# HaSai666/rec_pangu

Hardware: AMD Instinct MI355X
Metric: samples/sec DeepFM Criteo-shape bsz=65536/GPU (train step: fwd+bwd+dense Adam+zero_grad) (higher is better)
Workload: dtype f32

## Files before the change

### rec_pangu_amd/csrc/embed.hip

```cpp
#include "common.h"
#include <cstdlib>
#include "bfsplit.h"

struct IdxPtrs {
    const int64_t *p[RP_MAX_FIELDS];
};
struct DensePtrs {
    const float *p[RP_MAX_FIELDS];
};

template <int VEC>
struct Vec;
template <>
struct Vec<4> {
    typedef f32x4 T;
    static __device__ __forceinline__ T load(const float *p) { return *reinterpret_cast<const f32x4 *>(p); }
    static __device__ __forceinline__ void store(float *p, T v) { *reinterpret_cast<f32x4 *>(p) = v; }
    static __device__ __forceinline__ T zero() { return f32x4{0.f, 0.f, 0.f, 0.f}; }
    static __device__ __forceinline__ float hsum(T v) { return (v.x + v.y) + (v.z + v.w); }
};
template <>
struct Vec<1> {
    typedef float T;
    static __device__ __forceinline__ T load(const float *p) { return *p; }
    static __device__ __forceinline__ void store(float *p, T v) { *p = v; }
    static __device__ __forceinline__ T zero() { return 0.f; }
    static __device__ __forceinline__ float hsum(T v) { return v; }
};

template <int TPR, int VEC>
__global__ __launch_bounds__(256) void embed_gather_fwd_kernel(
    const float *__restrict__ arena, const int64_t *__restrict__ row_base, const int64_t *__restrict__ row_count,
    IdxPtrs idx, int F, DensePtrs dense, int ND, int64_t B, int D, float *__restrict__ x, int64_t ldx,
    float *__restrict__ fm_out, float *__restrict__ sum_out, int32_t *__restrict__ keys_out,
    int32_t *__restrict__ err_flag) {
    typedef Vec<VEC> V;
    constexpr int SPB = 256 / TPR;
    const int t = threadIdx.x % TPR;
    const int64_t b = (int64_t)blockIdx.x * SPB + threadIdx.x / TPR;
    if (b >= B) return;
    float *xrow = x + b * ldx;
    float fm_acc = 0.f;
    for (int c = t * VEC; c < D; c += TPR * VEC) {
        typename V::T s = V::zero(), q = V::zero();
#pragma unroll 4
        for (int f = 0; f < F; ++f) {
            int64_t id = idx.p[f][b];
            if (id < 0 || id >= row_count[f]) {
                *err_flag = 1;
                id = 0;
            }
            const int64_t key = row_base[f] + id;
            const typename V::T v = V::load(arena + key * D + c);
            V::store(xrow + (int64_t)f * D + c, v);
            s += v;
            q += v * v;
            if (keys_out != nullptr && c == 0) keys_out[(int64_t)f * B + b] = (int32_t)key;
        }
        if (sum_out != nullptr) V::store(sum_out + b * D + c, s);
        fm_acc += V::hsum(s * s - q);
    }
    const int64_t dense0 = (int64_t)F * D;
    for (int j = t; j < ND; j += TPR) xrow[dense0 + j] = dense.p[j][b];
    for (int64_t j = dense0 + ND + t; j < ldx; j += TPR) xrow[j] = 0.f;
    if (fm_out != nullptr) {
#pragma unroll
        for (int o = TPR / 2; o > 0; o >>= 1) fm_acc += __shfl_xor(fm_acc, o, TPR);
        if (t == 0) fm_out[b] = 0.5f * fm_acc;
    }
}

#define RP_SEG 8
template <int TPR, int VEC, bool LEVEL1 = false, bool POOL = false>
__global__ __launch_bounds__(256) void embed_grad_reduce_kernel(
    const int32_t *__restrict__ sk, const int32_t *__restrict__ sp, int64_t n, int Bi, int D,
    const float *__restrict__ dx, int64_t ldx, const float *__restrict__ gfm, const float *__restrict__ sum_in,
    const float *__restrict__ arena, float *__restrict__ G, int accumulate, float *__restrict__ gpiece,
    int32_t *__restrict__ gkey, const int32_t *__restrict__ bag_of = nullptr, const float *__restrict__ scale = nullptr) {
    typedef Vec<VEC> V;
    constexpr int GPB = 256 / TPR;
    constexpr int W = TPR * VEC;
    __shared__ __attribute__((aligned(16))) float piece[GPB][2][W];
    __shared__ int32_t pkey[GPB][2];
    __shared__ int32_t pcont[GPB];
    const int t = threadIdx.x % TPR, grp = threadIdx.x / TPR;
    const int64_t start = ((int64_t)blockIdx.x * GPB + grp) * RP_SEG;
    const bool active = start < n;
    const int cnt = active ? (int)((n - start) < RP_SEG ? (n - start) : RP_SEG) : 0;
    int32_t k[RP_SEG];
    int bb[RP_SEG], ff[RP_SEG];
#pragma unroll
    for (int j = 0; j < RP_SEG; ++j) {
        const bool ok = j < cnt;
        k[j] = ok ? sk[start + j] : -1;
        if (LEVEL1) {
            ff[j] = 0;
            bb[j] = (int)(start + j);
        } else if (POOL) {
            const int32_t p = ok ? sp[start + j] : 0;
            ff[j] = 0;
            bb[j] = bag_of ? (ok ? bag_of[p] : 0) : p / Bi;
        } else {
            const int32_t p = ok ? sp[start + j] : 0;
            ff[j] = p / Bi;
            bb[j] = p - ff[j] * Bi;
        }
    }
    const int32_t kprev = (active && start > 0) ? sk[start - 1] : -1;
    const int32_t knext = (active && start + cnt < n) ? sk[start + cnt] : -1;
    if (LEVEL1) {
        bool any = false;
#pragma unroll
        for (int j = 0; j < RP_SEG; ++j) any |= k[j] >= 0;
        if (!__syncthreads_or((int)any)) {
            if (threadIdx.x == 0) {
                gkey[2 * (int64_t)blockIdx.x] = -1;
                gkey[2 * (int64_t)blockIdx.x + 1] = -1;
            }
            return;
        }
    }
    float *hp = gpiece + (int64_t)blockIdx.x * 2 * D, *tp = hp + D;
    for (int c0 = 0; c0 < D; c0 += W) {
        const int c = c0 + t * VEC;
        const bool col_ok = c < D;
        typename V::T r[RP_SEG], w[RP_SEG];
        float gf[RP_SEG];
#pragma unroll
        for (int j = 0; j < RP_SEG; ++j) {
            r[j] = V::zero();
            w[j] = V::zero();
            gf[j] = 0.f;
            if (j < cnt && col_ok && !(LEVEL1 && k[j] < 0)) {
                if (dx != nullptr) r[j] = V::load(dx + (int64_t)bb[j] * ldx + (int64_t)ff[j] * D + c);
                if (POOL && scale != nullptr) r[j] = r[j] * V::load(scale + (int64_t)bb[j] * D + c);
                if (gfm != nullptr) {
                    gf[j] = gfm[bb[j]];
                    if (sum_in != nullptr) r[j] += gf[j] * V::load(sum_in + (int64_t)bb[j] * D + c);
                    if (j + 1 >= cnt || k[j + 1] != k[j]) w[j] = V::load(arena + (int64_t)k[j] * D + c);
                }
            }
        }
        if (t == 0) {
            pkey[grp][0] = -1;
            pkey[grp][1] = -1;
            pcont[grp] = 0;
        }
        typename V::T acc = V::zero();
        float gs = 0.f;
        bool run_head = (k[0] != kprev);
#pragma unroll
        for (int j = 0; j < RP_SEG; ++j) {
            if (j < cnt) {
                acc += r[j];
                gs += gf[j];
                const bool last_of_run = (j + 1 < cnt) ? (k[j + 1] != k[j]) : true;
                if (last_of_run) {
                    const bool run_ends_here = (j + 1 < cnt) ? true : (k[j] != knext);
                    if (gfm != nullptr) acc -= gs * w[j];
                    if (LEVEL1 && k[j] < 0) {
                    } else if (run_head && run_ends_here) {
                        if (col_ok) {
                            float *dst = G + (int64_t)k[j] * D + c;
                            V::store(dst, accumulate ? V::load(dst) + acc : acc);
                        }
                    } else {
                        const int slot = run_head ? 1 : 0;
                        V::store(&piece[grp][slot][t * VEC], acc);
                        if (t == 0) {
                            pkey[grp][slot] = k[j];
                            if (!run_ends_here) pcont[grp] = 1;
                        }
                    }
                    acc = V::zero();
                    gs = 0.f;
                    run_head = true;
                }
            }
        }
        __syncthreads();
        if (grp == 0) {
            const bool head_open = pkey[0][0] >= 0;
            int last_g = -1;
            for (int g2 = GPB - 1; g2 >= 0; --g2)
                if (pkey[g2][0] >= 0 || pkey[g2][1] >= 0) {
                    last_g = g2;
                    break;
                }
            const int64_t wg_end = ((int64_t)blockIdx.x + 1) * GPB * RP_SEG;
            const int last_active = (int)(((n < wg_end ? n : wg_end) - (int64_t)blockIdx.x * GPB * RP_SEG + RP_SEG - 1) / RP_SEG) - 1;
            const bool tail_open = last_g >= 0 && last_g == last_active && pcont[last_g] != 0;
            int32_t cur = -1;
            bool cur_is_head = false;
            typename V::T cacc = V::zero();
            int32_t headkey = -1, tailkey = -1;
            typename V::T headv = V::zero(), tailv = V::zero();
            for (int g2 = 0; g2 < GPB; ++g2) {
#pragma unroll
                for (int slot = 0; slot < 2; ++slot) {
                    const int32_t key = pkey[g2][slot];
                    if (key < 0) continue;
                    const typename V::T pv = V::load(&piece[g2][slot][t * VEC]);
                    if (key == cur) {
                        cacc += pv;
                    } else {
                        if (cur >= 0) {
                            if (cur_is_head) {
                                headkey = cur;
                                headv = cacc;
                            } else if (col_ok) {
                                float *dst = G + (int64_t)cur * D + c;
                                V::store(dst, accumulate ? V::load(dst) + cacc : cacc);
                            }
                        }
                        cur = key;
                        cacc = pv;
                        cur_is_head = head_open && g2 == 0 && slot == 0;
                    }
                }
            }
            if (cur >= 0) {
                if (tail_open) {
                    if (cur_is_head) {
                        headkey = cur;
                        headv = cacc;
                        tailkey = cur;
                    } else {
                        tailkey = cur;
                        tailv = cacc;
                    }
                } else if (cur_is_head) {
                    headkey = cur;
                    headv = cacc;
                } else if (col_ok) {
                    float *dst = G + (int64_t)cur * D + c;
                    V::store(dst, accumulate ? V::load(dst) + cacc : cacc);
                }
            }
            if (col_ok) {
                V::store(hp + c, headv);
                V::store(tp + c, tailv);
            }
            if (t == 0 && c0 == 0) {
                gkey[2 * (int64_t)blockIdx.x] = headkey;
                gkey[2 * (int64_t)blockIdx.x + 1] = tailkey;
            }
        }
        __syncthreads();
    }
}

#define EG_LD 72
#define EG_CT 68
#define EGL_MAXF 32

#define EGL_XLD 68
#define EGL_KLD 33
template <bool FULL, bool STORE_X = true, bool BF16_ROWS = false>
__global__ __launch_bounds__(256, 2) void embed_gather_linear_kernel(
    const float *__restrict__ arena, const int64_t *__restrict__ row_base, const int64_t *__restrict__ row_count,
    IdxPtrs idx, int F, DensePtrs dense, int ND, int64_t B, int64_t blk0, float *__restrict__ x, int64_t ldx,
    const float *__restrict__ W, int64_t ldw, const float *__restrict__ bias, float *__restrict__ h1,
    float *__restrict__ fm_out, float *__restrict__ sum_out, int32_t *__restrict__ keys_out, int32_t *__restrict__ err_flag,
    float *__restrict__ xd) {
    constexpr int D = 64;
    __shared__ __attribute__((aligned(16))) __bf16 Wt[3][64][EG_LD];
    __shared__ __attribute__((aligned(16))) float Xs[128][EGL_XLD];
    __shared__ int32_t Ks[128][EGL_KLD];
    const int t = threadIdx.x;
    const int wv = t >> 6, l = t & 63, i = l & 31, h = l >> 5;
    const int64_t blk = blk0 + blockIdx.x;
    const int64_t b = blk * 128 + 32 * wv + i;
    const bool bok = FULL || b < B;
    const int64_t bc = bok ? b : B - 1;
    const int g = t >> 4, sub = t & 15;
    const int wd = t >> 2, wc = (t & 3) * 16;

    for (int f = h; f < F; f += 2) {
        int64_t id = idx.p[f][bc];
        if (id < 0 || id >= row_count[f]) {
            if (bok) *err_flag = 1;
            id = 0;
        }
        const int64_t key = row_base[f] + id;
        Ks[32 * wv + i][f] = (int32_t)key;
        if (keys_out != nullptr && bok) keys_out[(int64_t)f * B + b] = (int32_t)key;
    }
    __syncthreads();
    const int g8 = t >> 3, s8 = t & 7;
    auto row_of = [&](int u) { return BF16_ROWS ? g8 + 32 * (u >> 1) : g + 16 * u; };
    auto col_of = [&](int u) { return BF16_ROWS ? 8 * s8 + 4 * (u & 1) : 4 * sub; };
    auto load_rows = [&](int f, f32x4 (&v)[8]) {
        if (BF16_ROWS) {
#pragma unroll
            for (int u = 0; u < 4; ++u) {
                const uint4 w4 = *reinterpret_cast<const uint4 *>(reinterpret_cast<const uint16_t *>(arena) +
                                                                  (int64_t)Ks[g8 + 32 * u][f] * D + 8 * s8);
                v[2 * u] = f32x4{__uint_as_float(w4.x << 16), __uint_as_float(w4.x & 0xffff0000u),
                                 __uint_as_float(w4.y << 16), __uint_as_float(w4.y & 0xffff0000u)};
                v[2 * u + 1] = f32x4{__uint_as_float(w4.z << 16), __uint_as_float(w4.z & 0xffff0000u),
                                     __uint_as_float(w4.w << 16), __uint_as_float(w4.w & 0xffff0000u)};
            }
        } else {
#pragma unroll
            for (int u = 0; u < 8; ++u) v[u] = *reinterpret_cast<const f32x4 *>(arena + (int64_t)Ks[g + 16 * u][f] * D + 4 * sub);
        }
    };
    auto load_w = [&](int col0, f32x4 (&v)[4]) {
        const float *src = W + (int64_t)wd * ldw + col0 + wc;
#pragma unroll
        for (int u = 0; u < 4; ++u) v[u] = *reinterpret_cast<const f32x4 *>(src + 4 * u);
    };
    f32x16 acc[2];
#pragma unroll
    for (int nt = 0; nt < 2; ++nt)
#pragma unroll
        for (int r = 0; r < 16; ++r) acc[nt][r] = 0.f;
    f32x4 S[8];
    float q[8];
#pragma unroll
    for (int u = 0; u < 8; ++u) {
        S[u] = f32x4{0.f, 0.f, 0.f, 0.f};
        q[u] = 0.f;
    }
    f32x4 cur[8], nxt[8], wq[4], wqn[4];
    load_rows(0, cur);
    load_w(0, wq);
    for (int f = 0; f < F; ++f) {
        const int fn = f + 1 < F ? f + 1 : f;
        load_rows(fn, nxt);
        load_w(fn * D, wqn);
        __syncthreads();
#pragma unroll
        for (int u = 0; u < 8; ++u) {
            const int r = row_of(u);
            *reinterpret_cast<f32x4 *>(&Xs[r][col_of(u)]) = cur[u];
            const int64_t br = blk * 128 + r;
            if (STORE_X && (FULL || (x != nullptr && br < B))) {
                if (BF16_ROWS) {
                    uint2 w2;
                    w2.x = (__float_as_uint(cur[u][0]) >> 16) | (__float_as_uint(cur[u][1]) & 0xFFFF0000u);
                    w2.y = (__float_as_uint(cur[u][2]) >> 16) | (__float_as_uint(cur[u][3]) & 0xFFFF0000u);
                    *reinterpret_cast<uint2 *>(reinterpret_cast<uint16_t *>(x) + br * ldx + (int64_t)f * D + col_of(u)) = w2;
                } else {
                    *reinterpret_cast<f32x4 *>(x + br * ldx + (int64_t)f * D + col_of(u)) = cur[u];
                }
            }
            S[u] += cur[u];
#pragma unroll
            for (int e = 0; e < 4; ++e) q[u] = __builtin_fmaf(cur[u][e], cur[u][e], q[u]);
        }
#pragma unroll
        for (int u = 0; u < 2; ++u) {
            f32x8 v;
#pragma unroll
            for (int e = 0; e < 4; ++e) {
                v[e] = wq[2 * u][e];
                v[4 + e] = wq[2 * u + 1][e];
            }
            bf16x8 pc[3];
            bf_split8<3>(v, pc);
#pragma unroll
            for (int qq = 0; qq < 3; ++qq) *reinterpret_cast<bf16x8 *>(&Wt[qq][wd][wc + 8 * u]) = pc[qq];
        }
        __syncthreads();
#pragma unroll
        for (int ks = 0; ks < 4; ++ks) {
            const f32x4 v0 = *reinterpret_cast<const f32x4 *>(&Xs[32 * wv + i][ks * 16 + 8 * h]);
            const f32x4 v1 = *reinterpret_cast<const f32x4 *>(&Xs[32 * wv + i][ks * 16 + 8 * h + 4]);
            f32x8 av;
#pragma unroll
            for (int e = 0; e < 4; ++e) {
                av[e] = v0[e];
                av[4 + e] = v1[e];
            }
            bf16x8 a[3];
            bf_split8<3>(av, a);
#pragma unroll
            for (int nt = 0; nt < 2; ++nt) {
                bf16x8 bq[3];
#pragma unroll
                for (int qq = 0; qq < 3; ++qq) bq[qq] = *reinterpret_cast<const bf16x8 *>(&Wt[qq][nt * 32 + i][ks * 16 + 8 * h]);
#pragma unroll
                for (int pr = 0; pr < 6; ++pr) {
                    if (BF16_ROWS && BfProd<6>::pa(pr) != 0) continue;
                    acc[nt] = __builtin_amdgcn_mfma_f32_32x32x16_bf16(a[BfProd<6>::pa(pr)], bq[BfProd<6>::pb(pr)], acc[nt], 0, 0, 0);
                }
            }
        }
#pragma unroll
        for (int u = 0; u < 8; ++u) cur[u] = nxt[u];
#pragma unroll
        for (int u = 0; u < 4; ++u) wq[u] = wqn[u];
    }
    if (ND > 0) {
        __syncthreads();
        {
#pragma unroll
            for (int u = 0; u < 4; ++u) {
                const int e = (t & 3) * 4 + u;
                const float v = e < ND ? W[(int64_t)wd * ldw + (int64_t)F * D + e] : 0.f;
                const __bf16 hi = (__bf16)v;
                const float r1 = v - (float)hi;
                const __bf16 mid = (__bf16)r1;
                Wt[0][wd][e] = hi;
                Wt[1][wd][e] = mid;
                Wt[2][wd][e] = (__bf16)(r1 - (float)mid);
            }
        }
        f32x8 dv;
#pragma unroll
        for (int e = 0; e < 8; ++e) {
            const int k = 8 * h + e;
            dv[e] = k < ND ? dense.p[k][bc] : 0.f;
        }
        __syncthreads();
        if (x != nullptr && bok && BF16_ROWS) {
            uint16_t *xt = reinterpret_cast<uint16_t *>(x) + b * ldx + (int64_t)F * D;
#pragma unroll
            for (int e = 0; e < 8; ++e)
                if (8 * h + e < ND) {
                    uint32_t ub = __float_as_uint(dv[e]);
                    ub += 0x7FFFu + ((ub >> 16) & 1u);
                    xt[8 * h + e] = (uint16_t)(ub >> 16);
                }
            for (int64_t j = (int64_t)F * D + ND + h; j < ldx; j += 2) reinterpret_cast<uint16_t *>(x)[b * ldx + j] = 0;
        } else if (x != nullptr && bok) {
            float *xt = x + b * ldx + (int64_t)F * D;
#pragma unroll
            for (int e = 0; e < 8; ++e)
                if (8 * h + e < ND) xt[8 * h + e] = dv[e];
            for (int64_t j = (int64_t)F * D + ND + h; j < ldx; j += 2) x[b * ldx + j] = 0.f;
        }
        if (xd != nullptr && bok) {
            float *xt = xd + b * 64;
#pragma unroll
            for (int e = 0; e < 8; ++e) xt[8 * h + e] = (8 * h + e < ND) ? dv[e] : 0.f;
            for (int j = 16 + h; j < 64; j += 2) xt[j] = 0.f;
        }
        bf16x8 a[3];
        bf_split8<3>(dv, a);
#pragma unroll
        for (int nt = 0; nt < 2; ++nt) {
            bf16x8 bq[3];
#pragma unroll
            for (int qq = 0; qq < 3; ++qq) bq[qq] = *reinterpret_cast<const bf16x8 *>(&Wt[qq][nt * 32 + i][8 * h]);
#pragma unroll
            for (int pr = 0; pr < 6; ++pr)
                acc[nt] = __builtin_amdgcn_mfma_f32_32x32x16_bf16(a[BfProd<6>::pa(pr)], bq[BfProd<6>::pb(pr)], acc[nt], 0, 0, 0);
        }
    } else {
        if (x != nullptr && bok && BF16_ROWS)
            for (int64_t j = (int64_t)F * D + h; j < ldx; j += 2) reinterpret_cast<uint16_t *>(x)[b * ldx + j] = 0;
        else if (x != nullptr && bok)
            for (int64_t j = (int64_t)F * D + h; j < ldx; j += 2) x[b * ldx + j] = 0.f;
        if (xd != nullptr && bok)
            for (int j = h; j < 64; j += 2) xd[b * 64 + j] = 0.f;
    }
#pragma unroll
    for (int nt = 0; nt < 2; ++nt) {
        const int n = nt * 32 + i;
        const float bv = bias != nullptr ? bias[n] : 0.f;
#pragma unroll
        for (int r = 0; r < 16; ++r) {
            const int64_t m = blk * 128 + 32 * wv + (r & 3) + 8 * (r >> 2) + 4 * h;
            if (FULL || m < B) h1[m * 64 + n] = fmaxf(acc[nt][r] + bv, 0.f);
        }
    }
    if (BF16_ROWS) {
#pragma unroll
        for (int u = 0; u < 4; ++u) {
            const int64_t br = blk * 128 + g8 + 32 * u;
            float fmv = -(q[2 * u] + q[2 * u + 1]);
#pragma unroll
            for (int e = 0; e < 4; ++e) {
                fmv = __builtin_fmaf(S[2 * u][e], S[2 * u][e], fmv);
                fmv = __builtin_fmaf(S[2 * u + 1][e], S[2 * u + 1][e], fmv);
            }
            fmv += __shfl_xor(fmv, 1, 64);
            fmv += __shfl_xor(fmv, 2, 64);
            fmv += __shfl_xor(fmv, 4, 64);
            if ((FULL || br < B) && fm_out != nullptr && s8 == 0) fm_out[br] = 0.5f * fmv;
            if ((FULL || br < B) && sum_out != nullptr) {
                *reinterpret_cast<f32x4 *>(sum_out + br * D + 8 * s8) = S[2 * u];
                *reinterpret_cast<f32x4 *>(sum_out + br * D + 8 * s8 + 4) = S[2 * u + 1];
            }
        }
        return;
    }
#pragma unroll
    for (int u = 0; u < 8; ++u) {
        const int64_t br = blk * 128 + g + 16 * u;
        float fmv = -q[u];
#pragma unroll
        for (int e = 0; e < 4; ++e) fmv = __builtin_fmaf(S[u][e], S[u][e], fmv);
        fmv += __shfl_xor(fmv, 1, 64);
        fmv += __shfl_xor(fmv, 2, 64);
        fmv += __shfl_xor(fmv, 4, 64);
        fmv += __shfl_xor(fmv, 8, 64);
        if (FULL || br < B) {
            if (fm_out != nullptr && sub == 0) fm_out[br] = 0.5f * fmv;
            if (sum_out != nullptr) *reinterpret_cast<f32x4 *>(sum_out + br * D + 4 * sub) = S[u];
        }
    }
}

static int embed_gather_linear_launch(const float *arena, bool bf16_rows, const int64_t *row_base, const int64_t *row_count,
                                      const int64_t *const *idx_ptrs, int F, const float *const *dense_ptrs, int ND,
                                      int64_t B, int D, float *x, int64_t ldx, const float *W, int64_t ldw,
                                      const float *bias, float *h1, float *fm_out, float *sum_out, int32_t *keys_out,
                                      int32_t *err_flag, float *xd, rp_stream_t stream);

extern "C" int rp_embed_gather_linear_fits(int D, int ND, int hidden, int64_t ldx, int64_t ldw) {
    return (D == 64 && hidden == 64 && ND >= 0 && ND <= 16 && ldx % 4 == 0 && ldw % 4 == 0) ? 1 : 0;
}

extern "C" int rp_embed_gather_linear_fwd(const float *arena, const int64_t *row_base, const int64_t *row_count,
                                          const int64_t *const *idx_ptrs, int F, const float *const *dense_ptrs, int ND,
                                          int64_t B, int D, float *x, int64_t ldx, const float *W, int64_t ldw,
                                          const float *bias, float *h1, float *fm_out, float *sum_out, int32_t *keys_out,
                                          int32_t *err_flag, float *xd, rp_stream_t stream) {
    return embed_gather_linear_launch(arena, false, row_base, row_count, idx_ptrs, F, dense_ptrs, ND, B, D, x, ldx, W, ldw, bias,
                                      h1, fm_out, sum_out, keys_out, err_flag, xd, stream);
}

extern "C" int rp_embed_gather_linear_fwd_bf16(const void *arena_bf16, const int64_t *row_base, const int64_t *row_count,
                                               const int64_t *const *idx_ptrs, int F, const float *const *dense_ptrs, int ND,
                                               int64_t B, int D, const float *W, int64_t ldw, const float *bias, float *h1,
                                               float *fm_out, void *x_bf16, int64_t ldx, float *sum_out, int32_t *keys_out,
                                               int32_t *err_flag, float *xd, rp_stream_t stream) {
    RP_REQUIRE(x_bf16 == nullptr || (ldx % 4 == 0 && (reinterpret_cast<uintptr_t>(x_bf16) & 7u) == 0),
               "embed_gather_linear_fwd_bf16: the bf16 activation needs ldx %% 4 == 0 and 8-byte alignment");
    return embed_gather_linear_launch(reinterpret_cast<const float *>(arena_bf16), true, row_base, row_count, idx_ptrs, F,
                                      dense_ptrs, ND, B, D, reinterpret_cast<float *>(x_bf16), ldx, W, ldw, bias, h1, fm_out,
                                      sum_out, keys_out, err_flag, xd, stream);
}

static int embed_gather_linear_launch(const float *arena, bool bf16_rows, const int64_t *row_base, const int64_t *row_count,
                                      const int64_t *const *idx_ptrs, int F, const float *const *dense_ptrs, int ND,
                                      int64_t B, int D, float *x, int64_t ldx, const float *W, int64_t ldw,
                                      const float *bias, float *h1, float *fm_out, float *sum_out, int32_t *keys_out,
                                      int32_t *err_flag, float *xd, rp_stream_t stream) {
    RP_REQUIRE(arena && row_base && row_count && idx_ptrs && W && h1 && err_flag, "embed_gather_linear_fwd: null pointer");
    RP_REQUIRE(!(x && xd), "embed_gather_linear_fwd: give x (full activation) or xd (dense columns only), not both");
    RP_REQUIRE(F >= 1 && F <= RP_MAX_FIELDS && B >= 0, "embed_gather_linear_fwd: bad F/B");
    RP_REQUIRE(ND == 0 || dense_ptrs, "embed_gather_linear_fwd: dense_ptrs is null with ND=%d", ND);
    RP_REQUIRE((int64_t)F * B < (int64_t)INT32_MAX, "embed_gather_linear_fwd: F*B overflows int32 positions");
    if (F > EGL_MAXF || !rp_embed_gather_linear_fits(D, ND, 64, x ? ldx : 4, ldw) || !rp_aligned16(arena) || !rp_aligned16(W) ||
        (x && (!rp_aligned16(x) || ldx < (int64_t)F * D + ND)) || ldw < (int64_t)F * D + ND ||
        (sum_out && !rp_aligned16(sum_out)))
        return rp_fail(RP_ERR_UNSUPPORTED, "embed_gather_linear_fwd: needs D = 64, a 64-wide layer, ND <= 16, aligned operands");
    if (B == 0) return RP_OK;
    IdxPtrs ip;
    DensePtrs dp;
    for (int f = 0; f < F; ++f) {
        RP_REQUIRE(idx_ptrs[f], "embed_gather_linear_fwd: idx_ptrs[%d] is null", f);
        ip.p[f] = idx_ptrs[f];
    }
    for (int j = 0; j < ND; ++j) {
        RP_REQUIRE(dense_ptrs[j], "embed_gather_linear_fwd: dense_ptrs[%d] is null", j);
        dp.p[j] = dense_ptrs[j];
    }
    const int64_t nfull = B / 128;
    const int64_t nblk = rp_cdiv(B, 128);
    hipStream_t s = (hipStream_t)stream;
    if (bf16_rows) {
        if (nfull > 0 && x != nullptr)
            hipLaunchKernelGGL((embed_gather_linear_kernel<true, true, true>), dim3((unsigned)nfull), dim3(256), 0, s, arena,
                               row_base, row_count, ip, F, dp, ND, B, (int64_t)0, x, ldx, W, ldw, bias, h1, fm_out, sum_out,
                               keys_out, err_flag, xd);
        else if (nfull > 0)
            hipLaunchKernelGGL((embed_gather_linear_kernel<true, false, true>), dim3((unsigned)nfull), dim3(256), 0, s, arena,
                               row_base, row_count, ip, F, dp, ND, B, (int64_t)0, x, ldx, W, ldw, bias, h1, fm_out, sum_out,
                               keys_out, err_flag, xd);
        if (nblk > nfull)
            hipLaunchKernelGGL((embed_gather_linear_kernel<false, true, true>), dim3((unsigned)(nblk - nfull)), dim3(256), 0, s,
                               arena, row_base, row_count, ip, F, dp, ND, B, nfull, x, ldx, W, ldw, bias, h1, fm_out, sum_out,
                               keys_out, err_flag, xd);
        RP_LAUNCH_CHECK("embed_gather_linear_fwd (bf16 rows)");
        return RP_OK;
    }
    if (nfull > 0 && x != nullptr)
        hipLaunchKernelGGL((embed_gather_linear_kernel<true, true>), dim3((unsigned)nfull), dim3(256), 0, s, arena, row_base,
                           row_count, ip, F, dp, ND, B, (int64_t)0, x, ldx, W, ldw, bias, h1, fm_out, sum_out, keys_out, err_flag,
                           xd);
    else if (nfull > 0)
        hipLaunchKernelGGL((embed_gather_linear_kernel<true, false>), dim3((unsigned)nfull), dim3(256), 0, s, arena, row_base,
                           row_count, ip, F, dp, ND, B, (int64_t)0, x, ldx, W, ldw, bias, h1, fm_out, sum_out, keys_out, err_flag,
                           xd);
    if (nblk > nfull)
        hipLaunchKernelGGL((embed_gather_linear_kernel<false, true>), dim3((unsigned)(nblk - nfull)), dim3(256), 0, s, arena,
                           row_base, row_count, ip, F, dp, ND, B, nfull, x, ldx, W, ldw, bias, h1, fm_out, sum_out, keys_out,
                           err_flag, xd);
    RP_LAUNCH_CHECK("embed_gather_linear_fwd");
    return RP_OK;
}

#define EG_MAXG 34
struct GradRanges {
    int n;
    int64_t start[EG_MAXG], end[EG_MAXG];
    int tile0[EG_MAXG];
};

template <bool FM_U>
__global__ __launch_bounds__(256, 3) void embed_grad_gemm_kernel(
    const int32_t *__restrict__ sk, const int32_t *__restrict__ sp, int64_t n, int Bi, const float *__restrict__ dh,
    int64_t lddh, const float *__restrict__ wt, int64_t ldwt, const float *__restrict__ dx, int64_t ldx,
    const float *__restrict__ gfm, const float *__restrict__ sum_in, const float *__restrict__ arena,
    float *__restrict__ G, int accumulate, float *__restrict__ gpiece, int32_t *__restrict__ gkey, GradRanges rg) {
    typedef Vec<4> V;
    constexpr int D = 64, TPR = 16, VEC = 4, GPB = 16, W = 64;
    constexpr int SM_B = 3 * 64 * EG_LD * 2, SM_C = 128 * EG_CT * 4;
    __shared__ __attribute__((aligned(16))) char smem[SM_B > SM_C ? SM_B : SM_C];
    __shared__ __attribute__((aligned(16))) float piece[GPB][2][W];
    __shared__ int32_t pkey[GPB][2];
    __shared__ int32_t pcont[GPB];
    __shared__ int32_t tkey[130];
    __shared__ int32_t tsmp[128];
    __shared__ int32_t tfld[128];
    __shared__ float tgf[128];
    typedef __bf16(*BTile)[64][EG_LD];
    BTile Bt = reinterpret_cast<BTile>(smem);
    float(*Ct)[EG_CT] = reinterpret_cast<float(*)[EG_CT]>(smem);
    const int t = threadIdx.x % TPR, grp = threadIdx.x / TPR;
    int gi = 0;
    for (int g2 = 1; g2 < rg.n; ++g2)
        if ((int)blockIdx.x >= rg.tile0[g2]) gi = g2;
    const int64_t wg0 = rg.start[gi] + (int64_t)((int)blockIdx.x - rg.tile0[gi]) * GPB * RP_SEG;
    const int64_t gend = rg.end[gi];
    {
        const int wv = threadIdx.x >> 6, l = threadIdx.x & 63, i = l & 31, h = l >> 5;
        const int64_t prow = wg0 + 32 * wv + i;
        const bool rok = prow < gend;
        const int32_t pp = rok ? sp[prow] : 0;
        const int32_t kk = rok ? sk[prow] : -1;
        if (threadIdx.x == 0) tkey[0] = wg0 > 0 ? sk[wg0 - 1] : -1;
        if (threadIdx.x == 64) tkey[129] = wg0 + 128 < n ? sk[wg0 + 128] : -1;
        const int fr = pp / Bi, br = pp - fr * Bi;
        const int64_t plast = (wg0 + 127 < gend ? wg0 + 127 : gend - 1);
        const int f_lo = __builtin_amdgcn_readfirstlane(sp[wg0] / Bi), f_hi = __builtin_amdgcn_readfirstlane(sp[plast] / Bi);
        if (h == 0) {
            tkey[1 + 32 * wv + i] = kk;
            tsmp[32 * wv + i] = br;
            tfld[32 * wv + i] = fr;
        }
        const bool wrap = __syncthreads_or(rok && (fr < f_lo || fr > f_hi)) != 0;
        const float gme = (gfm != nullptr && rok) ? gfm[br] : 0.f;
        f32x4 araw[4][2];
        const float *asrc = dh + (int64_t)br * lddh + 8 * h;
#pragma unroll
        for (int ks = 0; ks < 4; ++ks) {
            araw[ks][0] = *reinterpret_cast<const f32x4 *>(asrc + ks * 16);
            araw[ks][1] = *reinterpret_cast<const f32x4 *>(asrc + ks * 16 + 4);
        }
        float uraw[2][16];
        if (FM_U) {
#pragma unroll
            for (int r = 0; r < 16; ++r) {
                const float *src = sum_in + (int64_t)tsmp[32 * wv + (r & 3) + 8 * (r >> 2) + 4 * h] * D + i;
                uraw[0][r] = src[0];
                uraw[1][r] = src[32];
            }
        }
        if (h == 0) tgf[32 * wv + i] = gme;
        f32x16 acc[2];
#pragma unroll
        for (int nt = 0; nt < 2; ++nt)
#pragma unroll
            for (int r = 0; r < 16; ++r) acc[nt][r] = 0.f;
        const int wd = threadIdx.x >> 2, wc = (threadIdx.x & 3) * 16;
        const int f_from = wrap ? 0 : f_lo, f_to = wrap ? (int)((n - 1) / Bi) : f_hi;
        bool first_pass = true, need_init = FM_U;
        for (int f = f_from; f <= f_to; ++f) {
            if (wrap && !__syncthreads_or(rok && fr == f)) continue;
            if (!first_pass) __syncthreads();
            first_pass = false;
            {
                const float *src = wt + ((int64_t)f * D + wd) * ldwt + wc;
#pragma unroll
                for (int u = 0; u < 2; ++u) {
                    const f32x4 v0 = *reinterpret_cast<const f32x4 *>(src + 8 * u), v1 = *reinterpret_cast<const f32x4 *>(src + 8 * u + 4);
                    f32x8 v;
#pragma unroll
                    for (int e = 0; e < 4; ++e) {
                        v[e] = v0[e];
                        v[4 + e] = v1[e];
                    }
                    bf16x8 pc[3];
                    bf_split8<3>(v, pc);
#pragma unroll
                    for (int q = 0; q < 3; ++q) *reinterpret_cast<bf16x8 *>(&Bt[q][wd][wc + 8 * u]) = pc[q];
                }
            }
            __syncthreads();
            if (FM_U && need_init) {
// ... 986 lines not shown
```

Baseline: 87.56 million.

## Prefetch embedding rows two fields ahead with ping-pong registers in fused gather-GEMM

Restructures the per-field loop of the fused embedding gather plus first-layer GEMM kernel. Embedding rows are now prefetched two fields ahead using ping-pong register buffers (only for full blocks), and W is reloaded into the same registers right after it is split into LDS. Bf16 rows stay packed in registers and are widened just before use, which halves prefetch register cost. Scheduling barriers and register-pin asm keep the compiler from reordering loads across the MFMA section. The intent is to hide gather latency behind the MFMA work, at the price of more live registers and possibly lower occupancy.

```diff
diff --git a/rec_pangu_amd/csrc/embed.hip b/rec_pangu_amd/csrc/embed.hip
--- a/rec_pangu_amd/csrc/embed.hip
+++ b/rec_pangu_amd/csrc/embed.hip
@@ -288,22 +288,30 @@
     }
     __syncthreads();
     const int g8 = t >> 3, s8 = t & 7;
+    constexpr int NLD = BF16_ROWS ? 4 : 8;
     auto row_of = [&](int u) { return BF16_ROWS ? g8 + 32 * (u >> 1) : g + 16 * u; };
     auto col_of = [&](int u) { return BF16_ROWS ? 8 * s8 + 4 * (u & 1) : 4 * sub; };
     auto load_rows = [&](int f, f32x4 (&v)[8]) {
         if (BF16_ROWS) {
 #pragma unroll
-            for (int u = 0; u < 4; ++u) {
-                const uint4 w4 = *reinterpret_cast<const uint4 *>(reinterpret_cast<const uint16_t *>(arena) +
-                                                                  (int64_t)Ks[g8 + 32 * u][f] * D + 8 * s8);
-                v[2 * u] = f32x4{__uint_as_float(w4.x << 16), __uint_as_float(w4.x & 0xffff0000u),
-                                 __uint_as_float(w4.y << 16), __uint_as_float(w4.y & 0xffff0000u)};
-                v[2 * u + 1] = f32x4{__uint_as_float(w4.z << 16), __uint_as_float(w4.z & 0xffff0000u),
-                                     __uint_as_float(w4.w << 16), __uint_as_float(w4.w & 0xffff0000u)};
-            }
+            for (int u = 0; u < 4; ++u)
+                v[u] = *reinterpret_cast<const f32x4 *>(reinterpret_cast<const uint16_t *>(arena) +
+                                                        (int64_t)Ks[g8 + 32 * u][f] * D + 8 * s8);
         } else {
 #pragma unroll
             for (int u = 0; u < 8; ++u) v[u] = *reinterpret_cast<const f32x4 *>(arena + (int64_t)Ks[g + 16 * u][f] * D + 4 * sub);
+        }
+    };
+    auto widen = [&](const f32x4 (&v)[8], f32x4 (&c)[8]) {
+#pragma unroll
+        for (int u = 0; u < 8; ++u) {
+            if (BF16_ROWS) {
+                const uint32_t w0 = __float_as_uint(v[u >> 1][2 * (u & 1)]), w1 = __float_as_uint(v[u >> 1][2 * (u & 1) + 1]);
+                c[u] = f32x4{__uint_as_float(w0 << 16), __uint_as_float(w0 & 0xffff0000u), __uint_as_float(w1 << 16),
+                             __uint_as_float(w1 & 0xffff0000u)};
+            } else {
+                c[u] = v[u];
+            }
         }
     };
     auto load_w = [&](int col0, f32x4 (&v)[4]) {
@@ -323,47 +331,57 @@
         S[u] = f32x4{0.f, 0.f, 0.f, 0.f};
         q[u] = 0.f;
     }
-    f32x4 cur[8], nxt[8], wq[4], wqn[4];
-    load_rows(0, cur);
+    constexpr bool TWO_DEEP = FULL;
+    f32x4 ra[8], rb[8], wq[4];
+    load_rows(0, ra);
     load_w(0, wq);
-    for (int f = 0; f < F; ++f) {
-        const int fn = f + 1 < F ? f + 1 : f;
-        load_rows(fn, nxt);
-        load_w(fn * D, wqn);
+    if (TWO_DEEP) load_rows(1 < F ? 1 : F - 1, rb);
+    auto field = [&](int f, f32x4 (&cur)[8], f32x4 (&oth)[8]) {
+        const int f1 = f + 1 < F ? f + 1 : F - 1, f2 = f + 2 < F ? f + 2 : F - 1;
+        if (!TWO_DEEP) load_rows(f1, oth);
         __syncthreads();
+#pragma unroll
+        for (int u = 0; u < 2; ++u) {
+            f32x8 v;
+#pragma unroll
+            for (int e = 0; e < 4; ++e) {
+                v[e] = wq[2 * u][e];
+                v[4 + e] = wq[2 * u + 1][e];
+            }
+            bf16x8 pc[3];
+            bf_split8<3>(v, pc);
+#pragma unroll
+            for (int qq = 0; qq < 3; ++qq) *reinterpret_cast<bf16x8 *>(&Wt[qq][wd][wc + 8 * u]) = pc[qq];
+        }
+        load_w(f1 * D, wq);
+        if (TWO_DEEP) {
+#pragma unroll
+            for (int u = 0; u < NLD; ++u) asm volatile("" : "+v"(cur[u]));
+        }
+        f32x4 c[8];
+        widen(cur, c);
 #pragma unroll
         for (int u = 0; u < 8; ++u) {
             const int r = row_of(u);
-            *reinterpret_cast<f32x4 *>(&Xs[r][col_of(u)]) = cur[u];
+            *reinterpret_cast<f32x4 *>(&Xs[r][col_of(u)]) = c[u];
             const int64_t br = blk * 128 + r;
             if (STORE_X && (FULL || (x != nullptr && br < B))) {
                 if (BF16_ROWS) {
                     uint2 w2;
-                    w2.x = (__float_as_uint(cur[u][0]) >> 16) | (__float_as_uint(cur[u][1]) & 0xFFFF0000u);
-                    w2.y = (__float_as_uint(cur[u][2]) >> 16) | (__float_as_uint(cur[u][3]) & 0xFFFF0000u);
+                    w2.x = (__float_as_uint(c[u][0]) >> 16) | (__float_as_uint(c[u][1]) & 0xFFFF0000u);
+                    w2.y = (__float_as_uint(c[u][2]) >> 16) | (__float_as_uint(c[u][3]) & 0xFFFF0000u);
                     *reinterpret_cast<uint2 *>(reinterpret_cast<uint16_t *>(x) + br * ldx + (int64_t)f * D + col_of(u)) = w2;
                 } else {
-                    *reinterpret_cast<f32x4 *>(x + br * ldx + (int64_t)f * D + col_of(u)) = cur[u];
-                }
-            }
-            S[u] += cur[u];
-#pragma unroll
-            for (int e = 0; e < 4; ++e) q[u] = __builtin_fmaf(cur[u][e], cur[u][e], q[u]);
-        }
-#pragma unroll
-        for (int u = 0; u < 2; ++u) {
-            f32x8 v;
-#pragma unroll
-            for (int e = 0; e < 4; ++e) {
-                v[e] = wq[2 * u][e];
-                v[4 + e] = wq[2 * u + 1][e];
-            }
-            bf16x8 pc[3];
-            bf_split8<3>(v, pc);
-#pragma unroll
-            for (int qq = 0; qq < 3; ++qq) *reinterpret_cast<bf16x8 *>(&Wt[qq][wd][wc + 8 * u]) = pc[qq];
-        }
+                    *reinterpret_cast<f32x4 *>(x + br * ldx + (int64_t)f * D + col_of(u)) = c[u];
+                }
+            }
+            S[u] += c[u];
+#pragma unroll
+            for (int e = 0; e < 4; ++e) q[u] = __builtin_fmaf(c[u][e], c[u][e], q[u]);
+        }
+        if (TWO_DEEP) load_rows(f2, cur);
         __syncthreads();
+        __builtin_amdgcn_sched_barrier(0);
 #pragma unroll
         for (int ks = 0; ks < 4; ++ks) {
             const f32x4 v0 = *reinterpret_cast<const f32x4 *>(&Xs[32 * wv + i][ks * 16 + 8 * h]);
@@ -388,10 +406,21 @@
                 }
             }
         }
-#pragma unroll
-        for (int u = 0; u < 8; ++u) cur[u] = nxt[u];
-#pragma unroll
-        for (int u = 0; u < 4; ++u) wq[u] = wqn[u];
+        __builtin_amdgcn_sched_barrier(0);
+    };
+    if (TWO_DEEP) {
+        int f = 0;
+        for (; f + 1 < F; f += 2) {
+            field(f, ra, rb);
+            field(f + 1, rb, ra);
+        }
+        if (f < F) field(f, ra, rb);
+    } else {
+        for (int f = 0; f < F; ++f) {
+            field(f, ra, rb);
+#pragma unroll
+            for (int u = 0; u < NLD; ++u) ra[u] = rb[u];
+        }
     }
     if (ND > 0) {
         __syncthreads();
```

Result: no change. 87.47 million, median of 4 (-0.1%).
